# vliu15/3d-brain-tumor-segmentation

Measured on AMD Instinct MI355X. Metric: training volumes/sec (2ch x 128^3), higher is better.
Workload: dtype f32; 1 GPU; BASELINE configs[1]: 2ch x 128^3, batch 1 per GPU, fp32, full fwd+bwd with Dice+KL+L2 VAE loss + Dice metric + TF-form Adam; CLI-default model (base_filters=32, depth=4, groups=8, reduction=8; 42,174,773 params); parallelism=dp1, global_batch=1

## Files before the change

3d-brain-tumor-segmentation_amd/csrc/bts_internal.h:

```cpp
#pragma once
#include "../../include/bts_hip.h"

int bts_gn_finalize_partials_(const double* partial, float* mean, float* rstd, int NG, long B, double count, float eps,
                              hipStream_t stream);

bool bts_gn_slab_blocks_(int N, long V, int C, int G, int* B, long* span);

int bts_se_mlp_bwd_(const double* red, double* scratch, const float* gap, const float* h, const float* ch, const float* w1, const float* w2,
                    float* dw1, float* dw2, float* dwsp, float* dgap, int N, int B, long V, int F, int R, int accumulate_params,
                    hipStream_t stream);

int bts_wino_launch_(const float* x, const float* up, const float* bias, float* y, int N, int D, int H, int W, int Cin, int ldx,
                     int Cout, int ldy, int accum, double* gnp, int gnG, long* gn_B, void* ws, long ws_bytes, hipStream_t stream);
long bts_wino_workspace_(int N, int D, int H, int W, int Cin, int Cout);
int bts_w3_launch_(const float* x, const float* up3, const float* bias, float* y, int N, int D, int H, int W, int Cin, int ldx,
                   int Cout, int ldy, int accum, double* gnp, int gnG, long* gn_B, void* ws, long ws_bytes, hipStream_t stream);
long bts_w3_workspace_(int N, int D, int H, int W, int Cin, int Cout);
int bts_igemm_reduce_(const float* part, const float* bias, float* y, long nvox, int Cout, int Npad, int ldy, int ksplit,
                      int with_bias, int accum, hipStream_t stream);
int bts_se_mlp_bwd_sample_(const double* red, double* scratch, const float* h, const float* ch, const float* w1, const float* w2, float* dgap, int N,
                           long V, int F, int R, hipStream_t stream);
int bts_se_bwd_middle_(double* partial, double* red, double* scratch, const float* gap, const float* h, const float* ch, const float* w1,
                       const float* w2, float* dw1, float* dw2, float* dwsp, float* dgap, int N, int B, long V, int F, int R,
                       int accumulate_params, hipStream_t stream);

int bts_img_note_use_(const float* base, unsigned bit, hipStream_t stream);
int bts_img_ensure_(const float* base, unsigned bit, hipStream_t stream);
void bts_img_mark_used_(const float* base, unsigned bit);
```

3d-brain-tumor-segmentation_amd/csrc/conv_igemm.hip:

```cpp
#include <stdlib.h>
#include "common.h"
#include "bts_internal.h"

#define MAXSLOT 8

int bts_prof_on();
void bts_prof_begin(int sym, double flops, hipStream_t stream);
void bts_prof_end(hipStream_t stream);

struct IgemmParams {
  const float* x;
  const float* wp;
  const float* bias;
  float* y;
  int N, Di, Hi, Wi, Cin, ldx;
  int Do, Ho, Wo;
  int Cout, ldy, Npad, KG;
  int ODa, OHa, OWa;
  int os, ooz, ooy, oox;
  int s, loz, loy, lox;
  int IZ, IY, IX;
  int lgTX, lgTY, TZ;
  int ntz, nty, ntx;
  int ntaps, flags;
// ... 1150 lines not shown
    }
    __syncthreads();
    if (kg + 1 < p.KG) fetch(kg + 1);
    const float* wk = p.wp + kg * wstepKG;
#pragma unroll
    for (int r = 0; r < 9; ++r) {
      float w[3][2][CO * 4];
#pragma unroll
      for (int dx = 0; dx < 3; ++dx)
#pragma unroll
        for (int hh = 0; hh < 2; ++hh)
#pragma unroll
          for (int q = 0; q < CO * 4; ++q) w[dx][hh][q] = wk[(r * 3 + dx) * wstepTap + hh * p.Npad * 4 + q];
      f32x4 xv[3][2];
#pragma unroll
      for (int dx = 0; dx < 3; ++dx) {
        const float* src = lb + (((r / 3) * IY + r % 3) * IX + dx) * S;
        xv[dx][0] = *reinterpret_cast<const f32x4*>(src);
        xv[dx][1] = *reinterpret_cast<const f32x4*>(src + 4);
      }
      __builtin_amdgcn_sched_barrier(0);
#pragma unroll
      for (int dx = 0; dx < 3; ++dx)
#pragma unroll
        for (int hh = 0; hh < 2; ++hh)
#pragma unroll
          for (int c = 0; c < CO; ++c)
#pragma unroll
            for (int j = 0; j < 4; ++j) acc[c] = fmaf(xv[dx][hh][j], w[dx][hh][c * 4 + j], acc[c]);
      __builtin_amdgcn_sched_barrier(0);
    }
  }
  const int oz = tz * TZ + mz, oy = ty * TY + my, ox = tx * TX + mx;
  if (oz >= p.D || oy >= p.H || ox >= p.W) return;
  float* yrow = p.y + ((((long)n * p.D + oz) * p.H + oy) * p.W + ox) * (long)p.ldy;
#pragma unroll
  for (int c = 0; c < CO; ++c) {
    if (c < p.Cout) {
      float v = acc[c];
      if (p.flags & IG_FLAG_BIAS) v += p.bias[c];
      if (p.flags & IG_FLAG_SIGMOID) v = sigmoidf_(v);
      if (p.flags & IG_FLAG_ACCUM) v += yrow[c];
      yrow[c] = v;
    }
  }
}

static int launch_dsc(const float* x, const float* wp, const float* bias, float* y, int N, int D, int H, int W, int Cin, int ldx,
                      int Cout, int ldy, int flags, hipStream_t stream) {
  if (Cout > 4 || (Cin & 7) || (ldx & 3) || (((uintptr_t)x) & 15)) return 1;
  const long tiles = (long)N * ((D + 1) / 2) * ((H + 3) / 4) * ((W + 31) / 32);
  const long min_tiles = getenv("BTS_IGEMM_DSC_MIN") ? atol(getenv("BTS_IGEMM_DSC_MIN")) : 1024;
  if (tiles < min_tiles || tiles > 0x7fffffffL) return 1;
  DscParams p;
  p.x = x; p.wp = wp; p.bias = bias; p.y = y;
  p.N = N; p.D = D; p.H = H; p.W = W; p.Cin = Cin; p.ldx = ldx; p.Cout = Cout; p.ldy = ldy;
  p.Npad = npad32(Cout); p.KG = Cin / 8;
  p.ntx = (W + 31) / 32; p.nty = (H + 3) / 4; p.ntz = (D + 1) / 2;
  p.flags = flags & (IG_FLAG_BIAS | IG_FLAG_ACCUM | IG_FLAG_SIGMOID);
  const bool prof = bts_prof_on();
  if (prof) bts_prof_begin(22, 2.0 * 27.0 * Cin * (double)Cout * (double)N * D * H * W, stream);
  (void)hipGetLastError();
  if (Cout <= 2) hipLaunchKernelGGL(dsc_kernel<2>, dim3((unsigned)tiles), dim3(256), 0, stream, p);
  else hipLaunchKernelGGL(dsc_kernel<4>, dim3((unsigned)tiles), dim3(256), 0, stream, p);
  if (prof) bts_prof_end(stream);
  BTS_LAUNCH_CHECK();
  return BTS_OK;
}

struct C2Params {
  const float* x;
  const float* wp;
  const float* bias;
  float* y;
  const float* wp2;
  const float* bias2;
  float* y2;
  int N, D, H, W, ldx, Cout, ldy, ldy2, Npad;
  int ntz, nty, ntx;
  double* gnp;
  int gn_G, gn_zt;
};

template <bool F2>
__global__ __launch_bounds__(256, 2) void c2_kernel(const C2Params p) {
  __shared__ float lds[2 * 6 * 6 * 34 + 16];
  const int tid = threadIdx.x;
  const int lane = tid & 63;
  const int wave = __builtin_amdgcn_readfirstlane(tid >> 6);
  const int h = lane >> 5, l32 = lane & 31;
  int b = blockIdx.x;
  const int tx = b % p.ntx; b /= p.ntx;
  const int ty = b % p.nty; b /= p.nty;
  const int tz = b % p.ntz;
  const int n = b / p.ntz;
  const int oz0 = tz * 4, oy0 = ty * 4, ox0 = tx * 32;
  for (int e = tid; e < 6 * 6 * 34; e += 256) {
    const int vz = e / (6 * 34), r = e - vz * (6 * 34);
    const int vy = r / 34, vx = r - vy * 34;
    const int z = oz0 - 1 + vz, yy = oy0 - 1 + vy, xx = ox0 - 1 + vx;
    float v0 = 0.f, v1 = 0.f;
    if ((unsigned)z < (unsigned)p.D && (unsigned)yy < (unsigned)p.H && (unsigned)xx < (unsigned)p.W) {
      const float* s = p.x + ((((long)n * p.D + z) * p.H + yy) * p.W + xx) * (long)p.ldx;
      v0 = s[0]; v1 = s[1];
    }
    lds[e] = v0;
    lds[6 * 6 * 34 + e] = v1;
  }
  float wt[27];
#pragma unroll
  for (int t = 0; t < 27; ++t) wt[t] = p.wp[((long)t * 2 * p.Npad + l32) * 4 + h];
  float w2 = 0.f;
  if (F2) w2 = p.wp2[l32 * 4 + h];
  __syncthreads();
  f32x16 acc[4], acc2[F2 ? 4 : 1];
#pragma unroll
  for (int i = 0; i < 4; ++i)
#pragma unroll
    for (int r = 0; r < 16; ++r) { acc[i][r] = 0.f; if (F2) acc2[F2 ? i : 0][r] = 0.f; }
// ... 31 lines not shown
        if (co >= p.Cout) continue;
        f32x4 v = {acc[oy][4 * g], acc[oy][4 * g + 1], acc[oy][4 * g + 2], acc[oy][4 * g + 3]};
        if (p.bias) {
#pragma unroll
          for (int j = 0; j < 4; ++j) v[j] += p.bias[co + j];
        }
        if (p.gnp) {
#pragma unroll
          for (int j = 0; j < 4; ++j) { gn_s += v[j]; gn_q = fmaf(v[j], v[j], gn_q); }
        }
        *reinterpret_cast<f32x4*>(p.y + pix * p.ldy + co) = v;
        if (F2) {
          f32x4 v2 = {acc2[F2 ? oy : 0][4 * g], acc2[F2 ? oy : 0][4 * g + 1], acc2[F2 ? oy : 0][4 * g + 2], acc2[F2 ? oy : 0][4 * g + 3]};
          if (p.bias2) {
#pragma unroll
            for (int j = 0; j < 4; ++j) v2[j] += p.bias2[co + j];
          }
          *reinterpret_cast<f32x4*>(p.y2 + pix * p.ldy2 + co) = v2;
        }
      }
    }
  }
  if (p.gnp) {
    const double ds = wave_sum_f64((double)gn_s), dq = wave_sum_f64((double)gn_q);
    __syncthreads();
    double* sh = reinterpret_cast<double*>(lds);
    if (lane == 0) { sh[wave * 2] = ds; sh[wave * 2 + 1] = dq; }
    __syncthreads();
    if (tid == 0) {
      const int g = tz / p.gn_zt;
      const long B = (long)p.gn_zt * p.nty * p.ntx;
      const long b_ = ((long)(tz - g * p.gn_zt) * p.nty + ty) * p.ntx + tx;
      double* o = p.gnp + (((long)n * p.gn_G + g) * B + b_) * 2;
      o[0] = sh[0] + sh[2] + sh[4] + sh[6];
      o[1] = sh[1] + sh[3] + sh[5] + sh[7];
    }
  }
}

static int launch_c2(const float* x, const float* wp, const float* bias, float* y, int N, int D, int H, int W, int Cin, int ldx,
                     int Cout, int ldy, int flags, const float* wp2, const float* bias2, float* y2, int ldy2, double* gnp, int gnG,
                     long* gn_B, hipStream_t stream) {
  if (Cin != 2 || Cout > 32 || Cout % 4 != 0 || ldy % 4 != 0 || (((uintptr_t)y) & 15)) return 1;
  if (flags & (IG_FLAG_ACCUM | IG_FLAG_SIGMOID)) return 1;
  if (y2 != nullptr && (ldy2 % 4 != 0 || (((uintptr_t)y2) & 15))) return 1;
  C2Params p;
  p.x = x; p.wp = wp; p.bias = (flags & IG_FLAG_BIAS) ? bias : nullptr; p.y = y;
  p.wp2 = wp2; p.bias2 = bias2; p.y2 = y2;
  p.N = N; p.D = D; p.H = H; p.W = W; p.ldx = ldx; p.Cout = Cout; p.ldy = ldy; p.ldy2 = ldy2; p.Npad = npad32(Cout);
  p.ntz = (D + 3) / 4; p.nty = (H + 3) / 4; p.ntx = (W + 31) / 32;
  const long tiles = (long)N * p.ntz * p.nty * p.ntx;
  const long min_tiles = getenv("BTS_IGEMM_C2_MIN") ? atol(getenv("BTS_IGEMM_C2_MIN")) : 512;
  if (tiles < min_tiles || tiles > 0x7fffffffL) return 1;
  p.gnp = nullptr; p.gn_G = 0; p.gn_zt = 1;
  if (gnp != nullptr && gnG > 0 && D % gnG == 0 && (D / gnG) % 4 == 0 && getenv("BTS_IGEMM_NOGNFUSE") == nullptr) {
    p.gnp = gnp; p.gn_G = gnG; p.gn_zt = (D / gnG) / 4;
  }
  const bool prof = bts_prof_on();
  if (prof) bts_prof_begin(25, 2.0 * (27.0 + (y2 ? 1.0 : 0.0)) * Cin * (double)Cout * (double)N * D * H * W, stream);
  (void)hipGetLastError();
  if (y2 != nullptr) hipLaunchKernelGGL(c2_kernel<true>, dim3((unsigned)tiles), dim3(256), 0, stream, p);
  else hipLaunchKernelGGL(c2_kernel<false>, dim3((unsigned)tiles), dim3(256), 0, stream, p);
  if (prof) bts_prof_end(stream);
  BTS_LAUNCH_CHECK();
  if (gn_B && p.gnp != nullptr) *gn_B = (long)p.gn_zt * p.nty * p.ntx;
  return BTS_OK;
}

enum Geo { GEO_K1 = 0, GEO_S1 = 1, GEO_DOWN = 2, GEO_UP = 3 };

template <int MS, int NS, int WM, int WN, int KGS, bool FUSE2 = false, bool FIXG = false, bool T27 = false>
static int launch_cfg(IgemmParams& p, hipStream_t stream) {
  constexpr int S = KGS * 8 + 4;
  const int tileVox = p.IZ * p.IY * p.IX;
  if (tileVox * KGS * 2 > 256 * MAXSLOT) return BTS_ERR_SHAPE;
  const int nstages_all = (p.KG + KGS - 1) / KGS;
  const size_t shmem = (size_t)((nstages_all > 1 && !IG_TRI(MS, NS, KGS, FUSE2, FIXG)) ? 2 : 1) * tileVox * S * sizeof(float);
  auto kern = igemm_kernel<MS, NS, WM, WN, KGS, FUSE2, FIXG, T27>;
  static bool attr_done = false;
  if (!attr_done && !p.plan_only) {
    hipError_t e = hipFuncSetAttribute(reinterpret_cast<const void*>(kern), hipFuncAttributeMaxDynamicSharedMemorySize, 160 * 1024);
    if (e != hipSuccess) return (int)e;
    attr_done = true;
  }
  const int NT = 32 * NS * WN;
  dim3 grid(p.N * p.ntz * p.nty * p.ntx, (p.Npad + NT - 1) / NT, p.ncls > 1 ? p.ncls : 1);
  p.ksplit = 1;
  p.kg_per = p.KG;
  p.ws_need = 0;
  const long wgs = (long)grid.x * grid.y;
  const long sk_below = (KGS == 1) ? 512 : 192, sk_target = (KGS == 1) ? 512 : 384;
  if (!FUSE2 && p.ncls <= 1 && wgs < sk_below && p.KG >= 4 * KGS) {
    int ks = (int)((sk_target + wgs - 1) / wgs);
    const int maxks = p.KG / (2 * KGS);
    if (ks > maxks) ks = maxks;
    if (ks > 64) ks = 64;
    if (ks > 1) {
      int per = (p.KG + ks - 1) / ks;
      per = (per + KGS - 1) / KGS * KGS;
      ks = (p.KG + per - 1) / per;
      const long need = (long)ks * p.N * p.Do * p.Ho * p.Wo * p.Npad * 4;
      if (ks > 1 && (p.plan_only || (p.part != nullptr && p.ws_bytes >= need))) {
        p.ksplit = ks;
        p.kg_per = per;
        p.ws_need = need;
        grid.z = ks;
      }
    }
  }
  if (p.ksplit > 1) p.gnp = nullptr;
  p.gn_gridy = (int)grid.y;
  if (p.plan_only) return BTS_OK;
  const bool prof = bts_prof_on();
  if (prof) {
    constexpr int cfgid = (MS == 2 && NS == 1) ? 0 : (MS == 2 && NS == 2) ? 1 : (MS == 1 && NS == 2) ? 2 : (WN == 2) ? 3 : 4;
    const double taps = (p.ncls > 1) ? 27.0 : (double)p.ntaps;
    bts_prof_begin(cfgid + (KGS == 4 ? 8 : 0), 2.0 * taps * p.Cin * p.Cout * (double)p.N * p.Do * p.Ho * p.Wo, stream);
  }
  (void)hipGetLastError(); hipLaunchKernelGGL(kern, grid, dim3(256), shmem, stream, p);
  if (prof) bts_prof_end(stream);
  BTS_LAUNCH_CHECK();
  if (p.ksplit > 1) {
    const long nvox = (long)p.N * p.Do * p.Ho * p.Wo;
    long blocks = (nvox * p.Cout + 255) / 256;
    if (blocks > 4096) blocks = 4096;
    (void)hipGetLastError(); hipLaunchKernelGGL(igemm_reduce_kernel, dim3((int)blocks), dim3(256), 0, stream, p.part, p.bias, p.y, nvox, p.Cout,
                       p.Npad, p.ldy, p.ksplit, p.flags);
    BTS_LAUNCH_CHECK();
  }
  return BTS_OK;
}

static int ilog2(int v) { int l = 0; while ((1 << l) < v) ++l; return l; }

static int choose_cfg(int geo, int N, int Do, int Ho, int Wo, int Npad, int* Mout) {
  const long vox = (long)Do * Ho * Wo;
  int M, cfg;
  if (geo == GEO_DOWN) {
    M = 64;
    cfg = (Npad >= 128) ? 2 : 3;
  } else {
    const long wg256 = (long)N * ((vox + 255) / 256) * ((Npad + 63) / 64);
    if (Npad <= 32) {
      if ((long)N * ((vox + 255) / 256) >= 512) { M = 256; cfg = 0; }
      else { M = 128; cfg = 4; }
    } else if (wg256 >= 512) { M = 256; cfg = 1; }
    else {
      M = 64;
      const long wg64_128 = (long)N * ((vox + 63) / 64) * ((Npad + 127) / 128);
      cfg = (Npad >= 128 && wg64_128 >= 384) ? 2 : 3;
    }
  }
  *Mout = M;
  return cfg;
}

static int launch_igemm(int geo, const float* x, const float* wp, const float* bias, float* y, int N, int Di, int Hi,
                        int Wi, int Cin, int ldx, int Do, int Ho, int Wo, int Cout, int ldy, int ODa, int OHa, int OWa,
                        int pz, int py, int px, int flags, hipStream_t stream, void* ws = nullptr, long ws_bytes = 0,
                        long* need_out = nullptr, const float* wp2 = nullptr, const float* bias2 = nullptr,
                        float* y2 = nullptr, int ldy2 = 0, double* gnp = nullptr, int gnG = 0, long* gn_B = nullptr,
                        const float* x2 = nullptr, int ldx2 = 0) {
  if (gn_B) *gn_B = 0;
  if (geo == GEO_S1 && wp2 == nullptr && need_out == nullptr && Cout <= 4) {
    { const int e = bts_img_ensure_(wp, 1u, stream); if (e != BTS_OK) return e; }
    const int r = launch_dsc(x, wp, bias, y, N, Di, Hi, Wi, Cin, ldx, Cout, ldy, flags, stream);
    if (r != 1) { bts_img_mark_used_(wp, 1u); return r; }
  }
  if (geo == GEO_S1 && need_out == nullptr && Cin == 2 && x2 == nullptr && (wp2 == nullptr) == (y2 == nullptr)) {
    { const int e = bts_img_ensure_(wp, 1u, stream); if (e != BTS_OK) return e; }
    const int r = launch_c2(x, wp, bias, y, N, Di, Hi, Wi, Cin, ldx, Cout, ldy, flags, wp2, bias2, y2, ldy2, gnp, gnG, gn_B, stream);
    if (r != 1) { bts_img_mark_used_(wp, 1u); return r; }
  }
  if (geo == GEO_S1 && need_out == nullptr && !(flags & IG_FLAG_SIGMOID)) {
    const long pairs = (long)((Cin + 7) / 8) * 2 * npad32(Cout) * 4;
    const float* up = wp + 27L * pairs;
    int r = bts_w3_launch_(x, up + 48L * pairs, (flags & IG_FLAG_BIAS) ? bias : nullptr, y, N, Di, Hi, Wi, Cin, ldx, Cout, ldy,
                           (flags & IG_FLAG_ACCUM) ? 1 : 0, gnp, gnG, gn_B, ws, ws_bytes, stream);
    if (r == 1)
      r = bts_wino_launch_(x, up, (flags & IG_FLAG_BIAS) ? bias : nullptr, y, N, Di, Hi, Wi, Cin, ldx, Cout, ldy,
                           (flags & IG_FLAG_ACCUM) ? 1 : 0, gnp, gnG, gn_B, ws, ws_bytes, stream);
    if (r == BTS_OK) {
      if (y2 != nullptr)
        return launch_igemm(GEO_K1, x, wp2, bias2, y2, N, Di, Hi, Wi, Cin, ldx, Di, Hi, Wi, Cout, ldy2, Di, Hi, Wi, 0, 0, 0,
                            bias2 ? IG_FLAG_BIAS : 0, stream);
      if (x2 != nullptr)
        return launch_igemm(GEO_K1, x2, wp2, nullptr, y, N, Di, Hi, Wi, Cin, ldx2, Di, Hi, Wi, Cout, ldy, Di, Hi, Wi, 0, 0, 0,
                            IG_FLAG_ACCUM, stream);
      return BTS_OK;
    }
    if (r != 1) return r;
  }
  if (geo == GEO_K1 && wp2 == nullptr && need_out == nullptr) {
    const int r = launch_k1s(x, wp, bias, y, (long)N * Di * Hi * Wi, Cin, ldx, Cout, ldy, flags, stream);
    if (r != 1) return r;
  }
  if (geo == GEO_UP && pz < 0 && wp2 == nullptr && !(flags & ~(IG_FLAG_BIAS | IG_FLAG_ACCUM | IG_FLAG_SIGMOID | IG_FLAG_VECIN | IG_FLAG_VECOUT))) {
    if (need_out != nullptr) {
      UpmParams pp;
      long need = 0;
      if (plan_upm(pp, N, Di, Hi, Wi, Cin, Cout, &need) && need > 0) { *need_out = need; return BTS_OK; }
    } else {
      const int r = launch_upm(x, wp, bias, y, N, Di, Hi, Wi, Cin, ldx, Cout, ldy, flags, ws, ws_bytes, stream);
      if (r != 1) return r;
    }
  }
  if (geo == GEO_S1 && need_out == nullptr) {
    const int e = bts_img_note_use_(wp, 1u, stream);
    if (e != BTS_OK) return e;
  }
  IgemmParams p;
  p.wp2 = wp2; p.bias2 = bias2; p.y2 = y2; p.ldy2 = ldy2;
  p.x2 = x2; p.ldx2 = ldx2;
  p.part = reinterpret_cast<float*>(ws);
  p.ws_bytes = ws_bytes;
  p.plan_only = need_out != nullptr;
  p.ws_need = 0;
  p.x = x; p.wp = wp; p.bias = bias; p.y = y;
  p.N = N; p.Di = Di; p.Hi = Hi; p.Wi = Wi; p.Cin = Cin; p.ldx = ldx;
  p.Do = Do; p.Ho = Ho; p.Wo = Wo; p.Cout = Cout; p.ldy = ldy;
  p.Npad = npad32(Cout); p.KG = (Cin + 7) / 8;
  p.ODa = ODa; p.OHa = OHa; p.OWa = OWa;
  p.os = 1; p.ooz = p.ooy = p.oox = 0;
  p.s = 1;
  p.flags = flags;
  if ((ldx % 4 == 0) && (Cin % 4 == 0) && (((uintptr_t)x) % 16 == 0)) p.flags |= IG_FLAG_VECIN;
  if ((ldy % 4 == 0) && (Cout % 4 == 0) && (((uintptr_t)y) % 16 == 0)) p.flags |= IG_FLAG_VECOUT;

  int offz[27], offy[27], offx[27], tw[27], nt = 0;
  int lo[3] = {0, 0, 0}, hi[3] = {0, 0, 0};
  if (geo == GEO_K1) {
    offz[0] = offy[0] = offx[0] = 0; tw[0] = 0; nt = 1;
  } else if (geo == GEO_S1) {
    for (int t = 0; t < 27; ++t) { offz[t] = t / 9 - 1; offy[t] = (t / 3) % 3 - 1; offx[t] = t % 3 - 1; tw[t] = t; }
    nt = 27;
    lo[0] = lo[1] = lo[2] = -1; hi[0] = hi[1] = hi[2] = 1;
  } else if (geo == GEO_DOWN) {
    for (int t = 0; t < 27; ++t) { offz[t] = t / 9; offy[t] = (t / 3) % 3; offx[t] = t % 3; tw[t] = t; }
    nt = 27;
    hi[0] = hi[1] = hi[2] = 2;
    p.s = 2;
  } else if (pz < 0) {
    lo[0] = lo[1] = lo[2] = -1;
    p.os = 2;
    nt = 8;
  } else {
    const int par[3] = {pz, py, px};
    int kz[2], ky[2], kx[2], dz[2], dy[2], dx[2], nz, ny, nx;
    auto axis = [](int pp, int* k, int* d) {
      if (pp == 0) { k[0] = 0; d[0] = 0; k[1] = 2; d[1] = -1; return 2; }
      k[0] = 1; d[0] = 0; return 1;
    };
    nz = axis(par[0], kz, dz); ny = axis(par[1], ky, dy); nx = axis(par[2], kx, dx);
    for (int a = 0; a < nz; ++a)
      for (int bb = 0; bb < ny; ++bb)
        for (int c = 0; c < nx; ++c) {
          offz[nt] = dz[a]; offy[nt] = dy[bb]; offx[nt] = dx[c];
          tw[nt] = (kz[a] * 3 + ky[bb]) * 3 + kx[c];
// ... 52 lines not shown
            p.cls_tw[c][ct] = (k[0][a] * 3 + k[1][bb]) * 3 + k[2][cc];
            ++ct;
          }
      p.cls_nt[c] = ct;
      for (; ct < 8; ++ct) { p.cls_tl[c][ct] = 0; p.cls_tw[c][ct] = 0; }
    }
  }

  int rc;
  const bool fixg = (geo == GEO_S1) && p.IX == 34 && p.IY == 6;
  if (fixg && !k1 && (cfg == 0 || cfg == 1)) {
    if (p.y2 != nullptr) {
      if (cfg == 0) rc = launch_cfg<2, 1, 4, 1, 1, true, true>(p, stream);
      else rc = BTS_ERR_UNSUPPORTED;
    } else {
      if (cfg == 0) rc = launch_cfg<2, 1, 4, 1, 1, false, true>(p, stream);
      else rc = launch_cfg<2, 2, 4, 1, 1, false, true>(p, stream);
    }
  } else if (k1) {
    switch (cfg) {
      case 0: rc = launch_cfg<2, 1, 4, 1, 4>(p, stream); break;
      case 1: rc = launch_cfg<2, 2, 4, 1, 4>(p, stream); break;
      case 2: rc = launch_cfg<1, 2, 2, 2, 4>(p, stream); break;
      case 3: rc = launch_cfg<1, 1, 2, 2, 4>(p, stream); break;
      default: rc = launch_cfg<1, 1, 4, 1, 4>(p, stream); break;
    }
  } else if (p.y2 != nullptr) {
    switch (cfg) {
      case 0: rc = launch_cfg<2, 1, 4, 1, 1, true>(p, stream); break;
      case 2: rc = launch_cfg<1, 2, 2, 2, 1, true>(p, stream); break;
      case 3: rc = launch_cfg<1, 1, 2, 2, 1, true>(p, stream); break;
      case 4: rc = launch_cfg<1, 1, 4, 1, 1, true>(p, stream); break;
      default: rc = BTS_ERR_UNSUPPORTED; break;
    }
  } else if (p.ntaps == 27 && p.ncls <= 1) {
    switch (cfg) {
      case 0: rc = launch_cfg<2, 1, 4, 1, 1, false, false, true>(p, stream); break;
      case 1: rc = launch_cfg<2, 2, 4, 1, 1, false, false, true>(p, stream); break;
      case 2: rc = launch_cfg<1, 2, 2, 2, 1, false, false, true>(p, stream); break;
      case 3: rc = launch_cfg<1, 1, 2, 2, 1, false, false, true>(p, stream); break;
      default: rc = launch_cfg<1, 1, 4, 1, 1, false, false, true>(p, stream); break;
    }
  } else {
    switch (cfg) {
      case 0: rc = launch_cfg<2, 1, 4, 1, 1>(p, stream); break;
      case 1: rc = launch_cfg<2, 2, 4, 1, 1>(p, stream); break;
      case 2: rc = launch_cfg<1, 2, 2, 2, 1>(p, stream); break;
      case 3: rc = launch_cfg<1, 1, 2, 2, 1>(p, stream); break;
      default: rc = launch_cfg<1, 1, 4, 1, 1>(p, stream); break;
    }
  }
  if (need_out) {
    *need_out = p.ws_need;
    if (geo == GEO_S1) {
      const long wn = bts_wino_workspace_(N, Di, Hi, Wi, Cin, Cout);
      if (wn > *need_out) *need_out = wn;
      const long w3 = bts_w3_workspace_(N, Di, Hi, Wi, Cin, Cout);
      if (w3 > *need_out) *need_out = w3;
    }
  }
  if (gn_B && rc == BTS_OK && p.gnp != nullptr) *gn_B = (long)p.gn_zt * p.nty * p.ntx * p.gn_gridy;
  return rc;
}

static int geo_of_kind_fwd(int kind) {
  switch (kind) {
    case BTS_CONV_K1: return GEO_K1;
    case BTS_CONV_K3S1: return GEO_S1;
    case BTS_CONV_K3S2: return GEO_DOWN;
    default: return GEO_UP;
  }
}

static int conv_fwd_impl(int kind, const float* x, const float* wp_fwd, const float* bias, float* y, void* ws, long ws_bytes,
                         long* need_out, int N, int D, int H, int W, int Cin, int ldx, int Cout, int ldy, int flags,
                         hipStream_t stream) {
  if (N <= 0 || D <= 0 || H <= 0 || W <= 0 || Cin <= 0 || Cout <= 0 || ldx < Cin || ldy < Cout) return BTS_ERR_SHAPE;
  int f = 0;
  if (bias) f |= IG_FLAG_BIAS;
  if (flags & BTS_CONV_FLAG_SIGMOID) f |= IG_FLAG_SIGMOID;
  if (flags & BTS_CONV_FLAG_ACCUM) f |= IG_FLAG_ACCUM;
  const int geo = geo_of_kind_fwd(kind);
  if (geo == GEO_K1 || geo == GEO_S1)
    return launch_igemm(geo, x, wp_fwd, bias, y, N, D, H, W, Cin, ldx, D, H, W, Cout, ldy, D, H, W, 0, 0, 0, f, stream, ws,
                        ws_bytes, need_out);
  if (geo == GEO_DOWN) {
    if ((D | H | W) & 1) return BTS_ERR_SHAPE;
    return launch_igemm(geo, x, wp_fwd, bias, y, N, D, H, W, Cin, ldx, D / 2, H / 2, W / 2, Cout, ldy, D / 2, H / 2,
                        W / 2, 0, 0, 0, f, stream, ws, ws_bytes, need_out);
  }
  return launch_igemm(GEO_UP, x, wp_fwd, bias, y, N, D, H, W, Cin, ldx, D, H, W, Cout, ldy, 2 * D, 2 * H, 2 * W, -1, -1, -1,
                      f, stream, ws, ws_bytes, need_out);
}

extern "C" int bts_conv3d_fwd(int kind, const float* x, const float* wp_fwd, const float* bias, float* y, void* workspace,
                              long workspace_bytes, int N, int D, int H, int W, int Cin, int ldx, int Cout, int ldy,
                              int flags, hipStream_t stream) {
  return conv_fwd_impl(kind, x, wp_fwd, bias, y, workspace, workspace_bytes, nullptr, N, D, H, W, Cin, ldx, Cout, ldy, flags,
                       stream);
}
extern "C" long bts_conv3d_fwd_workspace(int kind, int N, int D, int H, int W, int Cin, int Cout) {
  long need = 0;
  if (conv_fwd_impl(kind, nullptr, nullptr, nullptr, nullptr, nullptr, 0, &need, N, D, H, W, Cin, Cin, Cout, Cout, 0,
                    nullptr) != BTS_OK)
    return -1;
  return need;
// ... 157 lines not shown
```

3d-brain-tumor-segmentation_amd/ops.py:

```python
import ctypes
import weakref

import torch

from ._lib import ERRORS, lib

K1, K3S1, K3S2, K3S2T = 0, 1, 2, 3
ROLE_FWD, ROLE_BWD = 0, 1
FLAG_SIGMOID, FLAG_ACCUM = 1, 2
GN_SLAB, GN_CHANNEL = 0, 1

_workspaces = {}

_CFG = {0: '2,1,4,1', 1: '2,2,4,1', 2: '1,2,2,2', 3: '1,1,2,2', 4: '1,1,4,1'}


_VARIANTS = {33: {1: '<0,5>', 2: '<0,4>', 3: '<1,5>', 4: '<1,4>'},
             32: {1: '<3x3x3>', 2: '<1x1x1>'}}


def kernel_symbol(sym, detail=False):
    var, sym = sym >> 16, sym & 0xffff
    if var and detail and sym in _VARIANTS:
        return kernel_symbol(sym) + _VARIANTS[sym].get(var, '<%d>' % var)
    if sym == 20:
        return 'upm_kernel'
    if sym == 21:
        return 'k1s_kernel'
    if sym == 22:
        return 'dsc_kernel'
    if sym == 23:
        return 'wino_kernel'
    if sym == 24:
        return 'wgw_kernel'
    if sym == 25:
        return 'c2_kernel'
    if sym == 26:
        return 'k1w_kernel'
    if sym == 27:
        return 'w3_kernel'
    if sym == 30:
        return 'lp_conv_s1_kernel'
    if sym == 31:
        return 'lp_conv_gather_kernel'
    if sym == 32:
        return 'lp_wgrad_kernel'
    if sym == 33:
        return 'lp_s1d_kernel'
    if sym == 34:
        return 'lp_k1_kernel'
    if sym == 35:
        return 'lp_up_kernel'
    if sym == 36:
        return 'lp_wgs_kernel'
    if sym == 37:
        return 'lp_wgd_kernel'
    if sym == 38:
        return 'lp_s1z_kernel'
    if sym == 39:
        return 'lp_s2t_kernel'
    if sym == 40:
        return 'lp_c2_kernel'
    if sym >= 100:
        return 'wgrad_kernel<%d,%d>' % ((sym - 100) >> 2, (sym - 100) & 3)
    return 'igemm_kernel<%s,%d>' % (_CFG[sym & 7], 4 if sym & 8 else 1)


def profile_enable(on):
    lib().call('bts_profile_enable', 1 if on else 0)


def profile_records(detail=False):
    L = lib()
    out = []
    sym, fl, ms = ctypes.c_int(), ctypes.c_double(), ctypes.c_float()
    for i in range(L._bts_profile_count()):
        L.call('bts_profile_get', i, ctypes.byref(sym), ctypes.byref(fl), ctypes.byref(ms))
        out.append((kernel_symbol(sym.value, detail), fl.value, ms.value))
    return out


def conv_bwd_data_pair(dy, wp_bwd, dy2, wp2_bwd, dx, accumulate):
    n, d, h, w, cin = dx.shape
    cout = dy.shape[4]
    nb = lib().query('bts_conv3d_bwd_data_pair_workspace', n, d, h, w, cin, cout)
    ws = workspace(nb, dy.device) if nb > 0 else None
    lib().call('bts_conv3d_bwd_data_pair', _p(dy), _p(wp_bwd), _p(dy2), _p(wp2_bwd), _p(dx), _p(ws), nb, n, d, h, w, cin,
               ld_of(dx), cout, ld_of(dy), ld_of(dy2), FLAG_ACCUM if accumulate else 0, _stream())
    return dx


def conv_flops(kind, n, d, h, w, cin, cout):
    v = n * d * h * w
# ... 610 lines not shown
```

include/bts_hip.h:

```cpp
#ifndef BTS_HIP_H
#define BTS_HIP_H
#include <stdint.h>
#ifdef __cplusplus
extern "C" {
#endif

typedef struct ihipStream_t* bts_stream_t;

#define BTS_OK 0
#define BTS_ERR_SHAPE (-1)
#define BTS_ERR_ALIGN (-2)
#define BTS_ERR_UNSUPPORTED (-3)
#define BTS_ERR_WORKSPACE (-4)
#define BTS_ERR_RCCL_BASE (-100)

#define BTS_CONV_K1 0
#define BTS_CONV_K3S1 1
#define BTS_CONV_K3S2 2
#define BTS_CONV_K3S2T 3
#define BTS_ROLE_FWD 0
#define BTS_ROLE_BWD_DATA 1
#define BTS_CONV_FLAG_SIGMOID 1
#define BTS_CONV_FLAG_ACCUM 2

#define BTS_GN_SLAB 0
#define BTS_GN_CHANNEL 1


long bts_conv_packed_floats(int kind, int role, int Cin, int Cout);
int bts_conv_pack(int kind, int role, const float* w, float* wp, int Cin_ref, int Cout, int Cin_slab, int dup_start,
                  int dup_shift, bts_stream_t stream);
long bts_conv_pack_desc_bytes(void);
long bts_conv_pack_desc(void* host_table, int index, long first_block, int kind, int role, const float* w, float* wp,
                        int Cin_ref, int Cout, int Cin_slab, int dup_start, int dup_shift);
int bts_conv_pack_batch(const void* table_dev, const void* table_host, int n, long total_blocks, bts_stream_t stream);
long bts_conv_pack_generation(void);
int bts_conv_pack_forget(const float* wp);
long bts_conv3d_fwd_workspace(int kind, int N, int D, int H, int W, int Cin, int Cout);
int bts_conv3d_fwd(int kind, const float* x, const float* wp_fwd, const float* bias, float* y, void* workspace,
                   long workspace_bytes, int N, int D, int H, int W, int Cin, int ldx, int Cout, int ldy, int flags,
                   bts_stream_t stream);
int bts_conv3d_fwd_can_fuse(int N, int D, int H, int W, int Cin, int Cout);
int bts_conv3d_fwd_fused2(const float* x, const float* wp_fwd, const float* bias, float* y, const float* wp2,
                          const float* bias2, float* y2, int N, int D, int H, int W, int Cin, int ldx, int Cout, int ldy,
                          int ldy2, bts_stream_t stream);
long bts_conv3d_bwd_data_workspace(int kind, int N, int D, int H, int W, int Cin, int Cout);
int bts_conv3d_bwd_data(int kind, const float* dy, const float* wp_bwd, float* dx, void* workspace, long workspace_bytes,
                        int N, int D, int H, int W, int Cin, int lddx, int Cout, int lddy, int flags, bts_stream_t stream);
int bts_conv3d_fwd_config(int kind, int N, int D, int H, int W, int Cin, int Cout);
int bts_conv3d_bwd_data_config(int kind, int N, int D, int H, int W, int Cin, int Cout);
long bts_conv3d_bwd_weight_workspace(int kind, int N, int D, int H, int W, int Cin, int Cout);
int bts_conv3d_bwd_weight(int kind, const float* x, const float* dy, float* dw, float* db, void* workspace,
                          long workspace_bytes, int N, int D, int H, int W, int Cin, int ldx, int Cout, int lddy,
                          int dup_start, int dup_shift, int accumulate, bts_stream_t stream);

long bts_gn_workspace(int N, long V, int C, int G, int mode);
long bts_gn_bwd_workspace(int N, long V, int C, int G, int mode);
int bts_gn_stats(const float* x, float* mean, float* rstd, void* workspace, long workspace_bytes, int N, long V, int C,
                 int G, int mode, float eps, bts_stream_t stream);
int bts_gn_apply(const float* x, float* y, const float* gamma, const float* beta, const float* mean, const float* rstd,
                 int N, long V, int C, int ldy, int G, int mode, int relu, bts_stream_t stream);
int bts_gn_bwd(const float* x, const float* dy, float* dx, const float* gamma, const float* beta, const float* mean,
               const float* rstd, float* dgamma, float* dbeta, void* workspace, long workspace_bytes, int N, long V, int C,
               int lddy, int G, int mode, int relu, int accumulate_params, bts_stream_t stream);

long bts_colsum_workspace(int N, long rows, int C);
int bts_colsum(const float* x, float* out, void* workspace, long workspace_bytes, int N, long rows, int C, int ld,
               float scale, int sum_over_n, int accumulate, bts_stream_t stream);
int bts_se_mlp_fwd(const float* gap, const float* w1, const float* w2, float* h, float* ch, int N, int F, int R,
                   bts_stream_t stream);
int bts_block_epilogue_fwd(const float* res, const float* c2, float* out, float* sp, const float* wsp, const float* ch,
                           const float* gamma, const float* beta, const float* mean, const float* rstd, int N, long V,
                           int F, int ldo, int G, int mode, bts_stream_t stream);
long bts_se_bwd_workspace(int N, long V, int F, int R);
int bts_se_bwd(const float* dout, const float* res, const float* sp, const float* gap, const float* h, const float* ch,
               const float* w1, const float* w2, const float* wsp, float* dres, float* ds, float* dgap, float* dw1,
               float* dw2, float* dwsp, void* workspace, long workspace_bytes, int N, long V, int F, int R, int lddo,
               int accumulate_params, bts_stream_t stream);

long bts_block_bwd_workspace(int N, long V, int F, int R, int G);
int bts_block_bwd(const float* dout, int lddo, const float* res, const float* c2, const float* sp, const float* gap, const float* h,
                  const float* ch, const float* w1, const float* w2, const float* wsp, const float* gamma, const float* beta,
                  const float* mean, const float* rstd, float* dres, float* dc2, float* ds, float* dgap, float* dw1, float* dw2,
                  float* dwsp, float* dgamma, float* dbeta, void* workspace, long workspace_bytes, int N, long V, int F, int R, int G,
                  int accumulate_gate_params, int accumulate_norm_params, bts_stream_t stream);

int bts_dropout_mask(uint8_t* mask, long n, float rate, uint64_t seed, bts_stream_t stream);
int bts_dropout_apply(const float* x, const uint8_t* mask, float* y, long n, float rate, bts_stream_t stream);
int bts_normal(float* out, long n, uint64_t seed, bts_stream_t stream);
int bts_vae_sample_fwd(const float* proj, const float* eps, float* z, int N, int L, bts_stream_t stream);
int bts_vae_sample_bwd(const float* proj, const float* eps, const float* dz, float* dproj, int N, int L, bts_stream_t stream);
int bts_fill(float* p, long n, float v, bts_stream_t stream);
int bts_axpy(float* y, const float* x, long n, float a, bts_stream_t stream);
int bts_add_strided(float* dst, const float* src, long rows, int C, int ldd, int lds_, int accumulate, bts_stream_t stream);
int bts_scalar_lincomb(float* out, const float* a, const float* b, float ca, float cb, bts_stream_t stream);
int bts_relu_bwd(const float* y, const float* dy, float* dx, long n, bts_stream_t stream);
int bts_sigmoid_bwd(const float* y, const float* dy, float* dx, long rows, int C, int ldy, int lddy, bts_stream_t stream);

long bts_dense_workspace(int N, int in, int out);
int bts_dense_fwd(const float* x, const float* w, const float* bias, float* y, void* workspace, long workspace_bytes, int N,
                  int in, int out, int relu, bts_stream_t stream);
int bts_dense_bwd(const float* x, const float* w, const float* g, float* dx, float* dw, float* db, int N, int in, int out,
                  int accumulate_dx, int accumulate_params, bts_stream_t stream);
// ... 186 lines not shown
```

Before: 27.21 volumes/s.

## Add dedicated MFMA kernel for stride-2 downsampling 3D convolutions

Adds a specialized stride-2 3x3x3 conv kernel. It stages a 17x9x9 input halo in LDS with a parity-split layout so that each of the 27 taps reads contiguous rows, prefetches the next channel group into registers, and uses fp32 MFMA. The kernel can split the K dimension and fuse GroupNorm statistics. It is routed ahead of the generic implicit-GEMM path for the downsampling geometry. Workspace sizing is extended, and the weight-image ensure/mark calls move inside the dsc and c2 launchers so they run only when those kernels actually launch. The risk is that the new kernel may be slower than the tuned generic path for some shapes, and split-K adds a reduction pass.

```diff
diff --git a/3d-brain-tumor-segmentation_amd/csrc/bts_internal.h b/3d-brain-tumor-segmentation_amd/csrc/bts_internal.h
--- a/3d-brain-tumor-segmentation_amd/csrc/bts_internal.h
+++ b/3d-brain-tumor-segmentation_amd/csrc/bts_internal.h
@@ -27,3 +27,14 @@
 int bts_img_note_use_(const float* base, unsigned bit, hipStream_t stream);
 int bts_img_ensure_(const float* base, unsigned bit, hipStream_t stream);
 void bts_img_mark_used_(const float* base, unsigned bit);
+
+struct BtsS2Plan {
+  int NB, gridy, ntz, nty, ntx;
+  int ksplit, kg_per;
+  long ws_need;
+  int gn_fused, gn_zt;
+};
+int bts_s2_accept_(int N, int D, int H, int W, int Cin, int ldx, int Cout, int ldy, int sigmoid, int aligned16, int gnG, BtsS2Plan* pl);
+int bts_s2_launch_(const float* x, const float* wp, const float* bias, float* y, int N, int D, int H, int W, int Cin, int ldx, int Cout,
+                   int ldy, int with_bias, int accum, int sigmoid, double* gnp, int gnG, long* gn_B, void* ws, long ws_bytes,
+                   hipStream_t stream);
diff --git a/3d-brain-tumor-segmentation_amd/csrc/conv_igemm.hip b/3d-brain-tumor-segmentation_amd/csrc/conv_igemm.hip
--- a/3d-brain-tumor-segmentation_amd/csrc/conv_igemm.hip
+++ b/3d-brain-tumor-segmentation_amd/csrc/conv_igemm.hip
@@ -1226,6 +1226,7 @@
   const long tiles = (long)N * ((D + 1) / 2) * ((H + 3) / 4) * ((W + 31) / 32);
   const long min_tiles = getenv("BTS_IGEMM_DSC_MIN") ? atol(getenv("BTS_IGEMM_DSC_MIN")) : 1024;
   if (tiles < min_tiles || tiles > 0x7fffffffL) return 1;
+  { const int e = bts_img_ensure_(wp, 1u, stream); if (e != BTS_OK) return e; }
   DscParams p;
   p.x = x; p.wp = wp; p.bias = bias; p.y = y;
   p.N = N; p.D = D; p.H = H; p.W = W; p.Cin = Cin; p.ldx = ldx; p.Cout = Cout; p.ldy = ldy;
@@ -1239,6 +1240,7 @@
   else hipLaunchKernelGGL(dsc_kernel<4>, dim3((unsigned)tiles), dim3(256), 0, stream, p);
   if (prof) bts_prof_end(stream);
   BTS_LAUNCH_CHECK();
+  bts_img_mark_used_(wp, 1u);
   return BTS_OK;
 }
 
@@ -1376,6 +1378,7 @@
   const long tiles = (long)N * p.ntz * p.nty * p.ntx;
   const long min_tiles = getenv("BTS_IGEMM_C2_MIN") ? atol(getenv("BTS_IGEMM_C2_MIN")) : 512;
   if (tiles < min_tiles || tiles > 0x7fffffffL) return 1;
+  { const int e = bts_img_ensure_(wp, 1u, stream); if (e != BTS_OK) return e; }
   p.gnp = nullptr; p.gn_G = 0; p.gn_zt = 1;
   if (gnp != nullptr && gnG > 0 && D % gnG == 0 && (D / gnG) % 4 == 0 && getenv("BTS_IGEMM_NOGNFUSE") == nullptr) {
     p.gnp = gnp; p.gn_G = gnG; p.gn_zt = (D / gnG) / 4;
@@ -1387,6 +1390,7 @@
   else hipLaunchKernelGGL(c2_kernel<false>, dim3((unsigned)tiles), dim3(256), 0, stream, p);
   if (prof) bts_prof_end(stream);
   BTS_LAUNCH_CHECK();
+  bts_img_mark_used_(wp, 1u);
   if (gn_B && p.gnp != nullptr) *gn_B = (long)p.gn_zt * p.nty * p.ntx;
   return BTS_OK;
 }
@@ -1487,14 +1491,12 @@
                         const float* x2 = nullptr, int ldx2 = 0) {
   if (gn_B) *gn_B = 0;
   if (geo == GEO_S1 && wp2 == nullptr && need_out == nullptr && Cout <= 4) {
-    { const int e = bts_img_ensure_(wp, 1u, stream); if (e != BTS_OK) return e; }
     const int r = launch_dsc(x, wp, bias, y, N, Di, Hi, Wi, Cin, ldx, Cout, ldy, flags, stream);
-    if (r != 1) { bts_img_mark_used_(wp, 1u); return r; }
+    if (r != 1) return r;
   }
   if (geo == GEO_S1 && need_out == nullptr && Cin == 2 && x2 == nullptr && (wp2 == nullptr) == (y2 == nullptr)) {
-    { const int e = bts_img_ensure_(wp, 1u, stream); if (e != BTS_OK) return e; }
     const int r = launch_c2(x, wp, bias, y, N, Di, Hi, Wi, Cin, ldx, Cout, ldy, flags, wp2, bias2, y2, ldy2, gnp, gnG, gn_B, stream);
-    if (r != 1) { bts_img_mark_used_(wp, 1u); return r; }
+    if (r != 1) return r;
   }
   if (geo == GEO_S1 && need_out == nullptr && !(flags & IG_FLAG_SIGMOID)) {
     const long pairs = (long)((Cin + 7) / 8) * 2 * npad32(Cout) * 4;
@@ -1528,6 +1530,13 @@
       const int r = launch_upm(x, wp, bias, y, N, Di, Hi, Wi, Cin, ldx, Cout, ldy, flags, ws, ws_bytes, stream);
       if (r != 1) return r;
     }
+  }
+  if (geo == GEO_DOWN && need_out == nullptr && wp2 == nullptr && x2 == nullptr) {
+    const bool gnw = gnp != nullptr && gnG > 0 && getenv("BTS_IGEMM_NOGNFUSE") == nullptr;
+    const int r = bts_s2_launch_(x, wp, bias, y, N, Di, Hi, Wi, Cin, ldx, Cout, ldy, (flags & IG_FLAG_BIAS) ? 1 : 0,
+                                 (flags & IG_FLAG_ACCUM) ? 1 : 0, (flags & IG_FLAG_SIGMOID) ? 1 : 0, gnw ? gnp : nullptr, gnG, gn_B, ws,
+                                 ws_bytes, stream);
+    if (r != 1) return r;
   }
   if (geo == GEO_S1 && need_out == nullptr) {
     const int e = bts_img_note_use_(wp, 1u, stream);
@@ -1686,6 +1695,10 @@
   }
   if (need_out) {
     *need_out = p.ws_need;
+    if (geo == GEO_DOWN) {
+      BtsS2Plan pl;
+      if (bts_s2_accept_(N, Di, Hi, Wi, Cin, ldx, Cout, ldy, 0, 1, 0, &pl) && pl.ws_need > *need_out) *need_out = pl.ws_need;
+    }
     if (geo == GEO_S1) {
       const long wn = bts_wino_workspace_(N, Di, Hi, Wi, Cin, Cout);
       if (wn > *need_out) *need_out = wn;
diff --git a/3d-brain-tumor-segmentation_amd/csrc/conv_s2.hip b/3d-brain-tumor-segmentation_amd/csrc/conv_s2.hip
--- /dev/null
+++ b/3d-brain-tumor-segmentation_amd/csrc/conv_s2.hip
@@ -0,0 +1,307 @@
+#include <stdlib.h>
+#include "common.h"
+#include "bts_internal.h"
+#include "wino_util.h"
+
+int bts_prof_on();
+void bts_prof_begin(int sym, double flops, hipStream_t stream);
+void bts_prof_end(hipStream_t stream);
+
+#define S2_S 8
+#define S2_ROW 136
+#define S2_PLANE (9 * S2_ROW)
+#define S2_LDS_DW (9 * S2_PLANE)
+#define S2_NVOX (17 * 9 * 9)
+#define S2_NSLOT 11
+
+struct S2Params {
+  const float* x;
+  const float* wp;
+  const float* bias;
+  float* y;
+  int N, Di, Hi, Wi, Cin, ldx;
+  int Do, Ho, Wo, Cout, ldy, Npad, KG;
+  int ntz, nty, ntx;
+  int with_bias, accum;
+  int ksplit, kg_per;
+  float* part;
+  double* gnp;
+  int gn_G, gn_zt;
+};
+
+__host__ __device__ constexpr int s2_lds_vox(int vz, int vy, int vx) {
+  return (vz * 9 + (vy & 1) * 5 + (vy >> 1)) * S2_ROW + ((vx & 1) * 9 + (vx >> 1)) * S2_S;
+}
+__host__ __device__ constexpr int s2_tap(int t) { return s2_lds_vox(t / 9, (t / 3) % 3, t % 3); }
+
+template <int NB>
+__global__ __launch_bounds__(256, 3) void s2_kernel(const S2Params p) {
+  extern __shared__ __attribute__((aligned(16))) float lds[];
+  const int tid = threadIdx.x;
+  const int lane = tid & 63;
+  const int wave = __builtin_amdgcn_readfirstlane(tid >> 6);
+  const int h = lane >> 5, l32 = lane & 31;
+  const int mx = l32 & 7, my = l32 >> 3;
+
+  int b = blockIdx.x;
+  const int tx = b % p.ntx; b /= p.ntx;
+  const int ty = b % p.nty; b /= p.nty;
+  const int tz = b % p.ntz;
+  const int n = b / p.ntz;
+  const int oz0 = tz * 4, oy0 = ty * 4, ox0 = tx * 8;
+  const int iz0 = oz0 * 2, iy0 = oy0 * 2, ix0 = ox0 * 2;
+
+  const float* xbase = p.x + ((((long)n * p.Di + iz0) * p.Hi + iy0) * p.Wi + ix0) * (long)p.ldx;
+  const __amdgpu_buffer_rsrc_t xr = __builtin_amdgcn_make_buffer_rsrc((void*)xbase, 0, 0x7fffffff, 0x00020000);
+  unsigned goff[S2_NSLOT];
+  int loff[S2_NSLOT];
+#pragma unroll
+  for (int i = 0; i < S2_NSLOT; ++i) {
+    const int e = tid + i * 256;
+    goff[i] = 0x80000000u;
+    loff[i] = -1;
+    if (e < 2 * S2_NVOX) {
+      const int vox = e >> 1, q = e & 1;
+      const int vz = (int)(((float)vox + 0.5f) * (1.0f / 153.0f));
+      const int r = vox - vz * 153;
+      const int vy = (int)(((float)r + 0.5f) * (1.0f / 17.0f));
+      const int vx = r - vy * 17;
+      loff[i] = s2_lds_vox(vz, vy, vx) + q * 4;
+      if (iz0 + vz < p.Di && iy0 + vy < p.Hi && ix0 + vx < p.Wi) goff[i] = (unsigned)(((vz * p.Hi + vy) * p.Wi + vx) * p.ldx + q * 4) * 4u;
+    }
+  }
+
+  const int bbase = (wave * 18 + my) * S2_ROW + mx * S2_S + h * 4;
+  int lane_woff[NB];
+#pragma unroll
+  for (int nb = 0; nb < NB; ++nb) {
+    int ncol = (blockIdx.y * NB + nb) * 32 + l32;
+    if (ncol >= p.Npad) ncol = p.Npad - 1;
+    lane_woff[nb] = (h * p.Npad + ncol) * 4;
+  }
+  f32x16 acc[NB];
+#pragma unroll
+  for (int nb = 0; nb < NB; ++nb)
+#pragma unroll
+    for (int r = 0; r < 16; ++r) acc[nb][r] = 0.f;
+
+  int kgBeg = 0, kgEnd = p.KG;
+  if (p.ksplit > 1) {
+    kgBeg = blockIdx.z * p.kg_per;
+    kgEnd = kgBeg + p.kg_per;
+    if (kgEnd > p.KG) kgEnd = p.KG;
+  }
+  const int wstepKG = 2 * p.Npad * 4;
+  const int wstepTap = p.KG * wstepKG;
+
+  f32x4 pre[S2_NSLOT];
+  auto fetch = [&](int kg) {
+#pragma unroll
+    for (int i = 0; i < S2_NSLOT; ++i) {
+      pre[i] = bufload(xr, goff[i], (unsigned)kg * 32u);
+    }
+  };
+  auto commit = [&]() {
+#pragma unroll
+    for (int i = 0; i < S2_NSLOT; ++i)
+      if (i + 1 < S2_NSLOT || loff[i] >= 0) *reinterpret_cast<f32x4*>(lds + loff[i]) = pre[i];
+  };
+
+  f32x4 a[3][NB];
+#pragma unroll
+  for (int q = 0; q < 2; ++q)
+#pragma unroll
+    for (int nb = 0; nb < NB; ++nb)
+      a[q][nb] = *reinterpret_cast<const f32x4*>((p.wp + (kgBeg * wstepKG + q * wstepTap)) + lane_woff[nb]);
+
+  fetch(kgBeg);
+  commit();
+  __syncthreads();
+
+  for (int kg = kgBeg; kg < kgEnd; ++kg) {
+    const bool more = (kg + 1) < kgEnd;
+    if (more) fetch(kg + 1);
+    const int wk = kg * wstepKG;
+    const float* lb = lds + bbase;
+    f32x4 bf[2];
+    bf[0] = *reinterpret_cast<const f32x4*>(lb + s2_tap(0));
+#pragma unroll
+    for (int t = 0; t < 27; ++t) {
+      if (t + 2 < 27) {
+#pragma unroll
+        for (int nb = 0; nb < NB; ++nb)
+          a[(t + 2) % 3][nb] = *reinterpret_cast<const f32x4*>((p.wp + (wk + (t + 2) * wstepTap)) + lane_woff[nb]);
+      } else if (more) {
+#pragma unroll
+        for (int nb = 0; nb < NB; ++nb)
+          a[(t + 2) % 3][nb] = *reinterpret_cast<const f32x4*>((p.wp + (wk + wstepKG + (t + 2 - 27) * wstepTap)) + lane_woff[nb]);
+      }
+      if (t + 1 < 27) bf[(t + 1) % 2] = *reinterpret_cast<const f32x4*>(lb + s2_tap(t + 1 < 27 ? t + 1 : 0));
+      __builtin_amdgcn_sched_barrier(0);
+#pragma unroll
+      for (int j = 0; j < 4; ++j)
+#pragma unroll
+        for (int nb = 0; nb < NB; ++nb)
+          acc[nb] = __builtin_amdgcn_mfma_f32_32x32x2f32(a[t % 3][nb][j], bf[t % 2][j], acc[nb], 0, 0, 0);
+      __builtin_amdgcn_sched_barrier(0);
+    }
+    __syncthreads();
+    if (more) commit();
+    __syncthreads();
+  }
+
+  const int oz = oz0 + wave, oy = oy0 + my, ox = ox0 + mx;
+  const bool inside = oz < p.Do && oy < p.Ho && ox < p.Wo;
+  const long v = (((long)n * p.Do + oz) * p.Ho + oy) * p.Wo + ox;
+
+  if (p.ksplit > 1) {
+    if (!inside) return;
+    const long nvox = (long)p.N * p.Do * p.Ho * p.Wo;
+    float* row = p.part + ((long)blockIdx.z * nvox + v) * p.Npad;
+#pragma unroll
+    for (int nb = 0; nb < NB; ++nb) {
+      const int cb = (blockIdx.y * NB + nb) * 32;
+      if (cb >= p.Npad) continue;
+#pragma unroll
+      for (int g = 0; g < 4; ++g) {
+        f32x4 v4 = {acc[nb][4 * g + 0], acc[nb][4 * g + 1], acc[nb][4 * g + 2], acc[nb][4 * g + 3]};
+        *reinterpret_cast<f32x4*>(row + cb + 8 * g + 4 * h) = v4;
+      }
+    }
+    return;
+  }
+
+  double gn_s = 0.0, gn_q = 0.0;
+  if (inside) {
+    float* yrow = p.y + v * p.ldy;
+#pragma unroll
+    for (int nb = 0; nb < NB; ++nb) {
+      const int cb = (blockIdx.y * NB + nb) * 32;
+      if (cb >= p.Cout) continue;
+      float bs = 0.f, bq = 0.f;
+#pragma unroll
+      for (int g = 0; g < 4; ++g) {
+        const int co = cb + 8 * g + 4 * h;
+        f32x4 r = {acc[nb][4 * g + 0], acc[nb][4 * g + 1], acc[nb][4 * g + 2], acc[nb][4 * g + 3]};
+        if (p.with_bias) {
+#pragma unroll
+          for (int j = 0; j < 4; ++j) r[j] += p.bias[co + j];
+        }
+        if (p.gnp) {
+#pragma unroll
+          for (int j = 0; j < 4; ++j) { bs += r[j]; bq = fmaf(r[j], r[j], bq); }
+        }
+        f32x4* dst = reinterpret_cast<f32x4*>(yrow + co);
+        if (p.accum) {
+          const f32x4 o = *dst;
+          r += o;
+        }
+        *dst = r;
+      }
+      gn_s += (double)bs;
+      gn_q += (double)bq;
+    }
+  }
+  if (p.gnp) {
+    const double ds = wave_sum_f64(gn_s), dq = wave_sum_f64(gn_q);
+    double* sh = reinterpret_cast<double*>(lds);
+    if (lane == 0) { sh[wave * 2] = ds; sh[wave * 2 + 1] = dq; }
+    __syncthreads();
+    if (tid == 0) {
+      const int g = tz / p.gn_zt;
+      const long B = (long)p.gn_zt * p.nty * p.ntx * gridDim.y;
+      const long b_ = (((long)(tz - g * p.gn_zt) * p.nty + ty) * p.ntx + tx) * gridDim.y + blockIdx.y;
+      double* o = p.gnp + (((long)n * p.gn_G + g) * B + b_) * 2;
+      o[0] = sh[0] + sh[2] + sh[4] + sh[6];
+      o[1] = sh[1] + sh[3] + sh[5] + sh[7];
+    }
+  }
+}
+
+int bts_s2_accept_(int N, int D, int H, int W, int Cin, int ldx, int Cout, int ldy, int sigmoid, int aligned16, int gnG, BtsS2Plan* pl) {
+  const char* sw = getenv("BTS_S2");
+  if (sw != nullptr && sw[0] == '0') return 0;
+  if (N <= 0 || D <= 0 || H <= 0 || W <= 0 || Cin <= 0 || Cout <= 0) return 0;
+  if ((D | H | W) & 1) return 0;
+  if (Cin % 8 != 0 || Cout % 32 != 0) return 0;
+  if (ldx < Cin || ldy < Cout || ldx % 4 != 0 || ldy % 4 != 0 || !aligned16 || sigmoid) return 0;
+  if ((9L * H * W * ldx + Cin) * 4 >= (1L << 31)) return 0;
+  const int Do = D / 2, Ho = H / 2, Wo = W / 2;
+  const long ntz = (Do + 3) / 4, nty = (Ho + 3) / 4, ntx = (Wo + 7) / 8;
+  const long tiles = N * ntz * nty * ntx;
+  if (tiles < 32 || tiles >= (1L << 31)) return 0;
+  const int Npad = Cout, KG = Cin / 8;
+  const int NB = (Npad >= 64) ? 2 : 1;
+  const int gridy = (Npad + 32 * NB - 1) / (32 * NB);
+  int ks = 1, per = KG;
+  const long wgs = tiles * gridy;
+  if (wgs < 512 && KG >= 4) {
+    ks = (int)((512 + wgs - 1) / wgs);
+    if (ks > KG / 2) ks = KG / 2;
+    if (ks > 64) ks = 64;
+    per = (KG + ks - 1) / ks;
+    ks = (KG + per - 1) / per;
+  }
+  if (ks > 1 && Npad < 128) return 0;
+  int gn = 0;
+  if (gnG > 0 && ks == 1) {
+    if (Do % gnG != 0 || (Do / gnG) % 4 != 0) return 0;
+    gn = 1;
+  }
+  pl->NB = NB; pl->gridy = gridy;
+  pl->ntz = (int)ntz; pl->nty = (int)nty; pl->ntx = (int)ntx;
+  pl->ksplit = ks; pl->kg_per = per;
+  pl->ws_need = ks > 1 ? (long)ks * N * Do * Ho * Wo * Npad * 4 : 0;
+  pl->gn_fused = gn;
+  pl->gn_zt = gn ? (Do / gnG) / 4 : 1;
+  return 1;
+}
+
+extern "C" int bts_conv_s2_plan(int N, int D, int H, int W, int Cin, int ldx, int Cout, int ldy, int aligned16, int gnG, long* ws_need,
+                                int* ksplit, int* gn_fused) {
+  BtsS2Plan pl;
+  if (!bts_s2_accept_(N, D, H, W, Cin, ldx, Cout, ldy, 0, aligned16, gnG, &pl)) return 0;
+  if (ws_need) *ws_need = pl.ws_need;
+  if (ksplit) *ksplit = pl.ksplit;
+  if (gn_fused) *gn_fused = pl.gn_fused;
+  return 1;
+}
+
+int bts_s2_launch_(const float* x, const float* wp, const float* bias, float* y, int N, int D, int H, int W, int Cin, int ldx, int Cout,
+                   int ldy, int with_bias, int accum, int sigmoid, double* gnp, int gnG, long* gn_B, void* ws, long ws_bytes,
+                   hipStream_t stream) {
+  const int al = ((((uintptr_t)x) | ((uintptr_t)y) | ((uintptr_t)wp)) & 15) == 0;
+  BtsS2Plan pl;
+  if (!bts_s2_accept_(N, D, H, W, Cin, ldx, Cout, ldy, sigmoid, al, gnp != nullptr ? gnG : 0, &pl)) return 1;
+  S2Params p;
+  p.x = x; p.wp = wp; p.bias = bias; p.y = y;
+  p.N = N; p.Di = D; p.Hi = H; p.Wi = W; p.Cin = Cin; p.ldx = ldx;
+  p.Do = D / 2; p.Ho = H / 2; p.Wo = W / 2; p.Cout = Cout; p.ldy = ldy; p.Npad = Cout; p.KG = Cin / 8;
+  p.ntz = pl.ntz; p.nty = pl.nty; p.ntx = pl.ntx;
+  p.with_bias = with_bias ? 1 : 0; p.accum = accum ? 1 : 0;
+  p.ksplit = pl.ksplit; p.kg_per = pl.kg_per;
+  p.part = reinterpret_cast<float*>(ws);
+  if (p.ksplit > 1 && (ws == nullptr || ws_bytes < pl.ws_need || (((uintptr_t)ws) & 15))) { p.ksplit = 1; p.kg_per = p.KG; }
+  p.gnp = (pl.gn_fused && p.ksplit == 1) ? gnp : nullptr;
+  p.gn_G = gnG; p.gn_zt = pl.gn_zt;
+  auto kern = pl.NB == 2 ? s2_kernel<2> : s2_kernel<1>;
+  static bool attr_done[3] = {false, false, false};
+  if (!attr_done[pl.NB]) {
+    hipError_t e = hipFuncSetAttribute(reinterpret_cast<const void*>(kern), hipFuncAttributeMaxDynamicSharedMemorySize, S2_LDS_DW * 4);
+    if (e != hipSuccess) return (int)e;
+    attr_done[pl.NB] = true;
+  }
+  const dim3 grid(N * pl.ntz * pl.nty * pl.ntx, pl.gridy, p.ksplit);
+  const bool prof = bts_prof_on();
+  if (prof) bts_prof_begin(28, 2.0 * 27.0 * Cin * (double)Cout * (double)N * p.Do * p.Ho * p.Wo, stream);
+  (void)hipGetLastError();
+  hipLaunchKernelGGL(kern, grid, dim3(256), S2_LDS_DW * 4, stream, p);
+  if (prof) bts_prof_end(stream);
+  BTS_LAUNCH_CHECK();
+  if (p.ksplit > 1) {
+    const int r = bts_igemm_reduce_(p.part, bias, y, (long)N * p.Do * p.Ho * p.Wo, Cout, p.Npad, ldy, p.ksplit, p.with_bias, p.accum, stream);
+    if (r != BTS_OK) return r;
+  }
+  if (gn_B) *gn_B = p.gnp ? (long)p.gn_zt * pl.nty * pl.ntx * pl.gridy : 0;
+  return BTS_OK;
+}
diff --git a/3d-brain-tumor-segmentation_amd/ops.py b/3d-brain-tumor-segmentation_amd/ops.py
--- a/3d-brain-tumor-segmentation_amd/ops.py
+++ b/3d-brain-tumor-segmentation_amd/ops.py
@@ -39,6 +39,8 @@
         return 'k1w_kernel'
     if sym == 27:
         return 'w3_kernel'
+    if sym == 28:
+        return 's2_kernel'
     if sym == 30:
         return 'lp_conv_s1_kernel'
     if sym == 31:
diff --git a/include/bts_hip.h b/include/bts_hip.h
--- a/include/bts_hip.h
+++ b/include/bts_hip.h
@@ -49,6 +49,8 @@
                         int N, int D, int H, int W, int Cin, int lddx, int Cout, int lddy, int flags, bts_stream_t stream);
 int bts_conv3d_fwd_config(int kind, int N, int D, int H, int W, int Cin, int Cout);
 int bts_conv3d_bwd_data_config(int kind, int N, int D, int H, int W, int Cin, int Cout);
+int bts_conv_s2_plan(int N, int D, int H, int W, int Cin, int ldx, int Cout, int ldy, int aligned16, int gnG, long* ws_need,
+                     int* ksplit, int* gn_fused);
 long bts_conv3d_bwd_weight_workspace(int kind, int N, int D, int H, int W, int Cin, int Cout);
 int bts_conv3d_bwd_weight(int kind, const float* x, const float* dy, float* dw, float* db, void* workspace,
                           long workspace_bytes, int N, int D, int H, int W, int Cin, int ldx, int Cout, int lddy,
```

Result: no change. 27.22 volumes/s, median of 6 (+0.1%).
